# YyzHarry/imbalanced-regression

Measured on NVIDIA H100. Metric: images/sec, higher is better.
Workload: dtype bf16

## Files before the change

### imbalanced-regression_b200/csrc/conv_igemm.cu

```cuda
#include <stdlib.h>
#include "common.cuh"
#include "tc.cuh"
#include "conv.cuh"

namespace dirb200 {
using namespace tc;

constexpr int BM = 128;
constexpr int BK = 64;
constexpr int kProducerThreads = 128;
constexpr int kThreads = 384;
constexpr int kMaxTaps = 25;
constexpr int kMaxSmemBytes = 232448;

struct IgemmParams {
  const __nv_bfloat16* src;
  int n, hs, ws, cs;
  int hm, wm;
  int kh, kw, stride, pad;
  int transposed;
  int cls_on, cls_py, cls_px, full_h, full_w;
  int ntaps_c;
  int tap_list[kMaxTaps];
  long long tap_eoff[kMaxTaps];
  unsigned short tap_r[kMaxTaps], tap_s[kMaxTaps];
  FastDiv fd_hw, fd_wm, fd_cpb, fd_kw, fd_ntiles, fd_persplit;
  int cpb;
  long long pixels;
  int num_kblocks;
  int kblocks_per_split;
  int total_chunks;
  int m_tiles, n_tiles;
  int num_tiles;
  int a_mode;
  int i2c_stride, i2c_lo;
  int ldc;
  void* out;
  float* stat_out;
  const float* epi_scale;
  const float* epi_shift;
  const __nv_bfloat16* epi_res;
  int epi_relu;
  const __nv_bfloat16* bst_y;
  const float* bst_scale;
  const float* bst_shift;
};

template <int BN, bool STAGED_EPI>
struct Cfg {
  static constexpr int kABytes = BM * BK * 2;
  static constexpr int kBBytes = BN * BK * 2;
  static constexpr int kStageBytes = kABytes + kBBytes;
  static constexpr int kStages = BN == 128 ? (STAGED_EPI ? 5 : 6) : 8;
  static constexpr int kBarOffset = kStages * kStageBytes;
  static constexpr int kStageRowBytes = BN * 2 + 16;
  static constexpr int kEpiWarpBytes = 16 * kStageRowBytes;
  static constexpr int kEpiOffset = kBarOffset + 256;
  static constexpr int kStatWarpBytes = 2 * BN * 4;
  static constexpr int kStatOffset = kEpiOffset + (STAGED_EPI ? 8 * kEpiWarpBytes : 0);
  static constexpr int kSmemBytes = kStatOffset + (STAGED_EPI ? 8 * kStatWarpBytes : 0) + 1024;
  static_assert(kSmemBytes <= kMaxSmemBytes, "shared memory budget");
};

__device__ __forceinline__ uint32_t pack_pixel(long long p, const IgemmParams& P) {
  if (p >= P.pixels) return 0u;
  uint32_t n, rem, y, x;
  P.fd_hw.divmod(static_cast<uint32_t>(p), n, rem);
  P.fd_wm.divmod(rem, y, x);
  return 0x80000000u | (n << 18) | (y << 9) | x;
}

struct RowPre {
  int nb, yb, xb;
};
__device__ __forceinline__ RowPre row_pre(const IgemmParams& P, uint32_t pk) {
  RowPre rp;
  const int n = (pk >> 18) & 0x1FFF;
  int y = (pk >> 9) & 0x1FF, x = pk & 0x1FF;
  if (P.cls_on) {
    y = 2 * y + P.cls_py;
    x = 2 * x + P.cls_px;
  }
  rp.nb = n * P.hs;
  if (!P.transposed) {
    rp.yb = y * P.stride - P.pad;
    rp.xb = x * P.stride - P.pad;
  } else {
    rp.yb = y + P.pad;
    rp.xb = x + P.pad;
  }
  if (!(pk >> 31)) rp.yb = -(1 << 28);
  return rp;
}

__device__ __forceinline__ const __nv_bfloat16* tap_source(const IgemmParams& P, const RowPre& rp, int r, int s,
                                                           int coff, bool& ok) {
  int hi, wi;
  ok = true;
  if (!P.transposed) {
    hi = rp.yb + r;
    wi = rp.xb + s;
  } else {
    hi = rp.yb - r;
    wi = rp.xb - s;
    if (P.stride == 2) {
      ok = ((hi | wi) & 1) == 0;
      hi >>= 1;
      wi >>= 1;
    }
  }
  ok = ok && static_cast<unsigned>(hi) < static_cast<unsigned>(P.hs) &&
       static_cast<unsigned>(wi) < static_cast<unsigned>(P.ws);
  return ok ? P.src + (static_cast<size_t>(rp.nb + hi) * P.ws + wi) * P.cs + coff : P.src;
}

template <int BN, bool WGRAD, bool STEM, bool ATMA = false, bool AFFINE = false, bool BSTAT = false>
__global__ void __launch_bounds__(kThreads, 1)
igemm_kernel(const __grid_constant__ CUtensorMap tmap_b, const __grid_constant__ CUtensorMap tmap_a,
             const IgemmParams P) {
  using C = Cfg<BN, !WGRAD>;
  static_assert(BN == 64 || BN == 128, "tile width: one m64n64 / m64n128 wgmma per warpgroup and k step");
  static_assert(!ATMA || !STEM, "TMA-fed A operand: not for the stem");
  static_assert(!AFFINE || (!WGRAD && !STEM), "folded-BN epilogue: non-stem fprop GEMMs only");
  static_assert(!BSTAT || (ATMA && !WGRAD && !AFFINE), "BN-backward moments in the epilogue: TMA-fed dgrad GEMMs only");
  extern __shared__ uint8_t smem_raw[];
  const uint32_t smem_base = (smem_u32(smem_raw) + 1023u) & ~1023u;
  uint8_t* const smem_gen = smem_raw + (smem_base - smem_u32(smem_raw));
  const uint32_t bar_base = smem_base + C::kBarOffset;
  auto a_addr = [&](int s) { return smem_base + s * C::kStageBytes; };
  auto b_addr = [&](int s) { return smem_base + s * C::kStageBytes + C::kABytes; };
  constexpr uint32_t nstages = C::kStages;
  auto full_bar = [&](int s) { return bar_base + 8u * s; };
  auto empty_bar = [&](int s) { return bar_base + 8u * (C::kStages + s); };
  const int warp = static_cast<int>(threadIdx.x >> 5), lane = threadIdx.x & 31;

  int tile_first, tile_end, tile_step, fixed_n = 0;
  if constexpr (WGRAD) {
    tile_first = blockIdx.x; tile_end = P.num_tiles; tile_step = gridDim.x;
  } else {
    uint32_t gi, nn;
    P.fd_ntiles.divmod(blockIdx.x, gi, nn);
    fixed_n = static_cast<int>(nn);
    tile_first = static_cast<int>(gi);
    tile_end = P.m_tiles;
    tile_step = static_cast<int>(P.fd_ntiles.div(gridDim.x - 1u - nn)) + 1;
  }
  auto decode_tile = [&](int t, int& split, int& m_tile, int& n_tile, int& kb_begin, int& nk) {
    if constexpr (WGRAD) {
      uint32_t sp, rem, mt, nt;
      P.fd_persplit.divmod(static_cast<uint32_t>(t), sp, rem);
      P.fd_ntiles.divmod(rem, mt, nt);
      split = static_cast<int>(sp);
      m_tile = static_cast<int>(mt);
      n_tile = static_cast<int>(nt);
      kb_begin = split * P.kblocks_per_split;
      const int kb_end = min(P.num_kblocks, kb_begin + P.kblocks_per_split);
      nk = max(0, kb_end - kb_begin);
    } else {
      split = 0;
      m_tile = t;
      n_tile = fixed_n;
      kb_begin = 0;
      nk = P.num_kblocks;
    }
  };

  if (threadIdx.x == 0) {
    for (int s = 0; s < C::kStages; ++s) {
      mbar_init(full_bar(s), ATMA ? 1 : kProducerThreads + 1);
      mbar_init(empty_bar(s), 8);
    }
    fence_barrier_init();
  }
  __syncthreads();

  if (warp < 4) {
    if constexpr (!ATMA) {
      const int j = lane & 7;
      const int q = lane >> 3;
      uint32_t rs = 0, rph = 0;
      for (int t = tile_first; t < tile_end; t += tile_step) {
        int split, m_tile, n_tile, kb_begin, nk;
        decode_tile(t, split, m_tile, n_tile, kb_begin, nk);
        const int n0 = n_tile * BN;
        long long off8[8];
        uint32_t mask8[8];
        int chunk_r = 0, chunk_s = 0, chunk_c0 = 0;
        bool chunk_ok = true;
        uint32_t tile_off = 0;
        if constexpr (!WGRAD) {
          const RowPre rp = row_pre(P, pack_pixel(static_cast<long long>(m_tile) * BM + warp * 32 + lane, P));
          const bool rvalid = rp.yb > -(1 << 27);
          int oy = rp.yb, ox = rp.xb;
          if (P.transposed && P.stride == 2) { oy >>= 1; ox >>= 1; }
          const long long my_off = (static_cast<long long>(rp.nb + oy) * P.ws + ox) * P.cs;
          uint32_t vy = 0, vx = 0;
          if (rvalid) {
            const int nky = P.kh, nkx = STEM ? 4 : P.kw;
            for (int r = 0; r < nky; ++r) {
              int h = P.transposed ? rp.yb - r : rp.yb + r;
              bool ok = true;
              if (P.transposed && P.stride == 2) { ok = (h & 1) == 0; h >>= 1; }
              vy |= (ok && static_cast<unsigned>(h) < static_cast<unsigned>(P.hs) ? 1u : 0u) << r;
// ... 89 lines not shown
            }
            unsigned long long rowaddr = myaddr;
            if constexpr (STEM)
              rowaddr = reinterpret_cast<unsigned long long>(
                  P.src + ((static_cast<long long>(rp.nb + rp.yb + chunk_r) * P.ws + rp.xb) * P.cs));
#pragma unroll
            for (int i = 0; i < 8; ++i) {
              const int row = 4 * i + q;
              const unsigned long long a = __shfl_sync(0xffffffffu, rowaddr, row);
              const uint32_t okb = __shfl_sync(0xffffffffu, okbits, row);
              const bool ok = STEM ? ((okb >> (j >> 1)) & 1u) : (okb & 1u);
              const __nv_bfloat16* src = reinterpret_cast<const __nv_bfloat16*>(a) + j * 8;
              cp_async16(dst_base + row * 128 + ((j ^ (row & 7)) << 4), ok ? src : P.src, ok ? 16u : 0u);
            }
          }
          if (warp == 0) {
            if (elect_one()) {
              mbar_arrive_expect_tx(full_bar(s), C::kBBytes);
              if constexpr (!WGRAD) {
                tma_load_2d(b_addr(s), &tmap_b, full_bar(s), kcoord * BK, n0);
              } else {
#pragma unroll
                for (int i = 0; i < BN / 64; ++i)
                  tma_load_2d(b_addr(s) + i * 8192, &tmap_b, full_bar(s), n0 + 64 * i, kb * 64);
              }
            }
            __syncwarp();
          }
          cp_async_mbar_arrive_noinc(full_bar(s));
        }
      }
    } else if (warp == 0) {
      uint32_t rs = 0, rph = 0;
      for (int t = tile_first; t < tile_end; t += tile_step) {
        int split, m_tile, n_tile, kb_begin, nk;
        decode_tile(t, split, m_tile, n_tile, kb_begin, nk);
        const int n0 = n_tile * BN;
        int tile_w0 = 0, tile_h0 = 0, tile_n0 = 0;
        if constexpr (!WGRAD) {
          if (P.a_mode == 2) {
            uint32_t tn, rem, y0, x0;
            P.fd_hw.divmod(static_cast<uint32_t>(m_tile) * BM, tn, rem);
            P.fd_wm.divmod(rem, y0, x0);
            tile_n0 = static_cast<int>(tn);
            tile_w0 = static_cast<int>(x0) * P.i2c_stride + P.i2c_lo;
            tile_h0 = static_cast<int>(y0) * P.i2c_stride + P.i2c_lo;
          }
        }
        int tc = 0, cb = 0;
        for (int it = 0; it < nk; ++it) {
          const int s = static_cast<int>(rs);
          mbar_wait(empty_bar(s), rph ^ 1u);
          if (++rs == nstages) { rs = 0; rph ^= 1u; }
          const int kb = kb_begin + it;
          if (elect_one()) {
            if constexpr (!WGRAD) {
              mbar_arrive_expect_tx(full_bar(s), C::kBBytes + C::kABytes);
              if (P.a_mode == 1)
                tma_load_2d(a_addr(s), &tmap_a, full_bar(s), kb * BK, m_tile * BM);
              else
                tma_load_im2col_4d(a_addr(s), &tmap_a, full_bar(s), cb * BK, tile_w0, tile_h0, tile_n0,
                                   P.tap_s[tc], P.tap_r[tc]);
              tma_load_2d(b_addr(s), &tmap_b, full_bar(s), (P.tap_list[tc] * P.cpb + cb) * BK, n0);
            } else {
              const int nchunks = min(2, P.total_chunks - 2 * m_tile);
              mbar_arrive_expect_tx(full_bar(s), C::kBBytes + nchunks * 8192);
// ... 3 lines not shown
              } else {
                uint32_t n0i, rem, y0, x0;
                P.fd_hw.divmod(static_cast<uint32_t>(kb) * 64u, n0i, rem);
                P.fd_wm.divmod(rem, y0, x0);
                for (int i = 0; i < nchunks; ++i) {
                  uint32_t tap, cbk, r, sx;
                  P.fd_cpb.divmod(static_cast<uint32_t>(2 * m_tile + i), tap, cbk);
                  P.fd_kw.divmod(tap, r, sx);
                  tma_load_im2col_4d(a_addr(s) + i * 8192, &tmap_a, full_bar(s), static_cast<int>(cbk) * 64,
                                     static_cast<int>(x0) * P.i2c_stride + P.i2c_lo,
                                     static_cast<int>(y0) * P.i2c_stride + P.i2c_lo, static_cast<int>(n0i),
                                     static_cast<uint16_t>(sx), static_cast<uint16_t>(r));
                }
              }
#pragma unroll
              for (int i = 0; i < BN / 64; ++i)
                tma_load_2d(b_addr(s) + i * 8192, &tmap_b, full_bar(s), n0 + 64 * i, kb * 64);
            }
          }
          if constexpr (!WGRAD) {
            if (++cb == P.cpb) { cb = 0; ++tc; }
          }
          __syncwarp();
        }
      }
    }
    return;
  }

  const int g = (warp >> 2) - 1;
  const int wq = warp & 3;
  const int ew = g * 4 + wq;
  const int fr = lane >> 2, fc = 2 * (lane & 3);
  float* const stat_sm = reinterpret_cast<float*>(smem_gen + C::kStatOffset) + ew * (2 * BN);
  if constexpr (!WGRAD) {
    if (P.stat_out != nullptr)
      for (int i = lane; i < 2 * BN; i += 32) stat_sm[i] = 0.f;
  }
  constexpr uint32_t kLbo = WGRAD ? 8192u : 16u;
  constexpr uint32_t kadv = WGRAD ? (2048u >> 4) : (32u >> 4);
  constexpr int kT = WGRAD ? 1 : 0;
  float acc[BN / 2];
  uint32_t rs = 0, rph = 0;
  for (int t = tile_first; t < tile_end; t += tile_step) {
    int split, m_tile, n_tile, kb_begin, nk;
    decode_tile(t, split, m_tile, n_tile, kb_begin, nk);
    int prev = 0;
    for (int it = 0; it < nk; ++it) {
      const int s = static_cast<int>(rs);
      mbar_wait(full_bar(s), rph);
      if (++rs == nstages) { rs = 0; rph ^= 1u; }
      if constexpr (!ATMA) fence_proxy_async();
      const uint64_t adesc = make_smem_desc(a_addr(s) + g * 8192, kLbo, 1024u);
      const uint64_t bdesc = make_smem_desc(b_addr(s), kLbo, 1024u);
      wgmma_fence_operands(acc);
      wgmma_fence();
#pragma unroll
      for (int k = 0; k < BK / 16; ++k)
        wgmma_bf16<BN, kT, kT>(acc, adesc + static_cast<uint64_t>(k * kadv), bdesc + static_cast<uint64_t>(k * kadv),
                               (it > 0 || k > 0) ? 1u : 0u);
      wgmma_commit();
      wgmma_fence_operands(acc);
      if (it > 0) {
        wgmma_wait<1>();
        if (lane == 0) mbar_arrive(empty_bar(prev));
      }
      prev = s;
    }
    wgmma_wait<0>();
    wgmma_fence_operands(acc);
    if (nk > 0 && lane == 0) mbar_arrive(empty_bar(prev));
    const int n0 = n_tile * BN;

    if constexpr (!WGRAD) {
      const uint32_t stage_base = smem_base + C::kEpiOffset + ew * C::kEpiWarpBytes;
      const bool relu_now = AFFINE && P.epi_relu && P.epi_res == nullptr;
#pragma unroll
      for (int j = 0; j < BN / 8; ++j) {
        const int col = 8 * j + fc;
        float v0 = acc[4 * j], v1 = acc[4 * j + 1], v2 = acc[4 * j + 2], v3 = acc[4 * j + 3];
        if constexpr (AFFINE) {
          const float2 a = __ldg(reinterpret_cast<const float2*>(P.epi_scale + n0 + col));
          const float2 b = __ldg(reinterpret_cast<const float2*>(P.epi_shift + n0 + col));
          v0 = fmaf(v0, a.x, b.x); v1 = fmaf(v1, a.y, b.y); v2 = fmaf(v2, a.x, b.x); v3 = fmaf(v3, a.y, b.y);
          if (relu_now) { v0 = fmaxf(v0, 0.f); v1 = fmaxf(v1, 0.f); v2 = fmaxf(v2, 0.f); v3 = fmaxf(v3, 0.f); }
        }
        __nv_bfloat162 h0 = __floats2bfloat162_rn(v0, v1), h1 = __floats2bfloat162_rn(v2, v3);
        asm volatile("st.shared.b32 [%0], %1;" ::"r"(stage_base + fr * C::kStageRowBytes + col * 2),
                     "r"(*reinterpret_cast<uint32_t*>(&h0)) : "memory");
        asm volatile("st.shared.b32 [%0], %1;" ::"r"(stage_base + (fr + 8) * C::kStageRowBytes + col * 2),
                     "r"(*reinterpret_cast<uint32_t*>(&h1)) : "memory");
      }
      __syncwarp();
      constexpr int kLanesPerRow = BN * 2 / 16;
      constexpr int kRowsPerIter = 32 / kLanesPerRow;
      constexpr int kIters = 16 / kRowsPerIter;
      const int sub = lane / kLanesPerRow, col16 = lane % kLanesPerRow;
      const long long p0 = static_cast<long long>(m_tile) * BM + g * 64 + wq * 16;
      __nv_bfloat16* out_cols = reinterpret_cast<__nv_bfloat16*>(P.out) + n0 + col16 * 8;
#pragma unroll
      for (int i = 0; i < kIters; ++i) {
        const int rl = i * kRowsPerIter + sub;
        const long long p = p0 + rl;
        int orow = (p < P.pixels && nk > 0) ? static_cast<int>(p) : -1;
        if (orow >= 0 && P.cls_on) {
          const uint32_t pk = pack_pixel(p, P);
          const int n = (pk >> 18) & 0x1FFF, yy = (pk >> 9) & 0x1FF, xx = pk & 0x1FF;
          orow = (n * P.full_h + 2 * yy + P.cls_py) * P.full_w + 2 * xx + P.cls_px;
        }
        if (orow >= 0) {
          uint4 val;
          asm volatile("ld.shared.v4.b32 {%0, %1, %2, %3}, [%4];"
                       : "=r"(val.x), "=r"(val.y), "=r"(val.z), "=r"(val.w)
                       : "r"(stage_base + rl * C::kStageRowBytes + col16 * 16));
          if constexpr (AFFINE) {
            if (P.epi_res != nullptr) {
              const uint4 rv = *reinterpret_cast<const uint4*>(P.epi_res + n0 + col16 * 8 + static_cast<long long>(orow) * P.ldc);
              uint32_t o[4] = {val.x, val.y, val.z, val.w};
              const uint32_t rr[4] = {rv.x, rv.y, rv.z, rv.w};
#pragma unroll
              for (int e = 0; e < 4; ++e) {
                float lo = __uint_as_float(o[e] << 16) + __uint_as_float(rr[e] << 16);
                float hi = __uint_as_float(o[e] & 0xffff0000u) + __uint_as_float(rr[e] & 0xffff0000u);
                if (P.epi_relu) { lo = fmaxf(lo, 0.f); hi = fmaxf(hi, 0.f); }
                __nv_bfloat162 h = __floats2bfloat162_rn(lo, hi);
                o[e] = *reinterpret_cast<uint32_t*>(&h);
              }
              val = make_uint4(o[0], o[1], o[2], o[3]);
            }
          }
          *reinterpret_cast<uint4*>(out_cols + static_cast<long long>(orow) * P.ldc) = val;
        }
      }
      if (BSTAT || P.stat_out != nullptr) {
#pragma unroll
        for (int h = 0; h < BN / 64; ++h) {
          const int col = 2 * (lane + 32 * h);
          float s0 = 0.f, s1 = 0.f, q0 = 0.f, q1 = 0.f;
          float2 bsc = make_float2(0.f, 0.f), bsh = bsc;
          if constexpr (BSTAT) {
            bsc = __ldg(reinterpret_cast<const float2*>(P.bst_scale + n0 + col));
            bsh = __ldg(reinterpret_cast<const float2*>(P.bst_shift + n0 + col));
          }
#pragma unroll
          for (int r = 0; r < 16; ++r) {
            uint32_t w;
            asm volatile("ld.shared.b32 %0, [%1];" : "=r"(w) : "r"(stage_base + r * C::kStageRowBytes + col * 2));
            float g0 = __uint_as_float(w << 16), g1 = __uint_as_float(w & 0xffff0000u);
            if constexpr (BSTAT) {
              const long long p = p0 + r;
              const uint32_t yw = p < P.pixels ? __ldg(reinterpret_cast<const unsigned int*>(P.bst_y + p * P.ldc + n0 + col)) : 0u;
              const float y0 = __uint_as_float(yw << 16), y1 = __uint_as_float(yw & 0xffff0000u);
              if (!(fmaf(y0, bsc.x, bsh.x) > 0.f)) g0 = 0.f;
              if (!(fmaf(y1, bsc.y, bsh.y) > 0.f)) g1 = 0.f;
              s0 += g0; s1 += g1;
              q0 = fmaf(g0, y0, q0); q1 = fmaf(g1, y1, q1);
            } else {
              s0 += g0; s1 += g1;
              q0 = fmaf(g0, g0, q0); q1 = fmaf(g1, g1, q1);
            }
          }
          stat_sm[col] += s0;
          stat_sm[col + 1] += s1;
          stat_sm[BN + col] += q0;
          stat_sm[BN + col + 1] += q1;
        }
      }
      __syncwarp();
    } else {
      const int ktot = P.total_chunks * 64;
      const int krow = m_tile * BM + g * 64 + wq * 16 + fr;
      float* out = reinterpret_cast<float*>(P.out) + (static_cast<size_t>(split) * P.ldc + n0) * ktot;
#pragma unroll
      for (int j = 0; j < BN / 8; ++j) {
        const size_t c0 = static_cast<size_t>(8 * j + fc) * ktot;
#pragma unroll
        for (int e = 0; e < 2; ++e) {
          if (krow < ktot) out[c0 + e * ktot + krow] = nk > 0 ? acc[4 * j + e] : 0.f;
          if (krow + 8 < ktot) out[c0 + e * ktot + krow + 8] = nk > 0 ? acc[4 * j + 2 + e] : 0.f;
        }
      }
    }
  }
  if constexpr (!WGRAD) {
    if (P.stat_out != nullptr) {
      asm volatile("bar.sync 1, 256;" ::: "memory");
      const float* all = reinterpret_cast<const float*>(smem_gen + C::kStatOffset);
      float* dst = P.stat_out + static_cast<size_t>(blockIdx.x) * 2 * P.ldc + fixed_n * BN;
      for (int o = static_cast<int>(threadIdx.x) - kProducerThreads; o < 2 * BN; o += kThreads - kProducerThreads) {
        const int k = o / BN, col = o - k * BN;
        const float v = ((all[o] + all[2 * BN + o]) + (all[4 * BN + o] + all[6 * BN + o])) +
                        ((all[8 * BN + o] + all[10 * BN + o]) + (all[12 * BN + o] + all[14 * BN + o]));
        dst[static_cast<size_t>(k) * P.ldc + col] = v;
      }
    }
  }
}

typedef CUresult (*EncodeTiledFn)(CUtensorMap*, CUtensorMapDataType, cuuint32_t, void*, const cuuint64_t*,
                                  const cuuint64_t*, const cuuint32_t*, const cuuint32_t*, CUtensorMapInterleave,
                                  CUtensorMapSwizzle, CUtensorMapL2promotion, CUtensorMapFloatOOBfill);

static EncodeTiledFn encode_fn() {
  static EncodeTiledFn fn = nullptr;
  if (!fn) {
    void* p = nullptr;
    cudaDriverEntryPointQueryResult q;
    if (cudaGetDriverEntryPoint("cuTensorMapEncodeTiled", &p, cudaEnableDefault, &q) == cudaSuccess &&
        q == cudaDriverEntryPointSuccess)
      fn = reinterpret_cast<EncodeTiledFn>(p);
  }
  return fn;
}

int make_tmap_bf16_2d(CUtensorMap* tm, const void* ptr, uint64_t inner, uint64_t outer, uint64_t row_stride_bytes,
                      uint32_t box_outer) {
  EncodeTiledFn fn = encode_fn();
  if (!fn) {
    set_error("cuTensorMapEncodeTiled entry point not available");
// ... 56 lines not shown
  Q.fd_hw = make_fastdiv(static_cast<uint32_t>(Q.hm * Q.wm));
  Q.fd_wm = make_fastdiv(static_cast<uint32_t>(Q.wm));
  Q.fd_cpb = make_fastdiv(static_cast<uint32_t>(Q.cpb > 0 ? Q.cpb : 1));
  Q.fd_kw = make_fastdiv(static_cast<uint32_t>(Q.kw > 0 ? Q.kw : 1));
  Q.fd_ntiles = make_fastdiv(static_cast<uint32_t>(Q.n_tiles > 0 ? Q.n_tiles : 1));
  Q.fd_persplit = make_fastdiv(static_cast<uint32_t>(Q.m_tiles * Q.n_tiles > 0 ? Q.m_tiles * Q.n_tiles : 1));
  const int nt = Q.ntaps_c < kMaxTaps ? Q.ntaps_c : kMaxTaps;
  for (int i = 0; i < kMaxTaps; ++i) {
    Q.tap_eoff[i] = 0;
    Q.tap_r[i] = Q.tap_s[i] = 0;
  }
  for (int i = 0; i < nt && Q.kw > 0; ++i) {
    const int tp = Q.tap_list[i];
    int r = tp / Q.kw, sx = tp - r * Q.kw;
    if (Q.transposed && Q.cls_on) {
      Q.tap_r[i] = static_cast<unsigned short>((Q.cls_py + Q.pad - r) / 2 - Q.i2c_lo);
      Q.tap_s[i] = static_cast<unsigned short>((Q.cls_px + Q.pad - sx) / 2 - Q.i2c_lo);
      r >>= 1; sx >>= 1;
      Q.tap_eoff[i] = -static_cast<long long>(r * Q.ws + sx) * Q.cs;
    } else if (Q.transposed) {
      Q.tap_r[i] = static_cast<unsigned short>(Q.kh - 1 - r);
      Q.tap_s[i] = static_cast<unsigned short>(Q.kw - 1 - sx);
      if (Q.stride == 2) { r >>= 1; sx >>= 1; }
      Q.tap_eoff[i] = -static_cast<long long>(r * Q.ws + sx) * Q.cs;
    } else {
      Q.tap_r[i] = static_cast<unsigned short>(r);
      Q.tap_s[i] = static_cast<unsigned short>(sx);
      Q.tap_eoff[i] = static_cast<long long>(r * Q.ws + sx) * Q.cs;
    }
  }
  return Q;
}

template <int BN, bool WGRAD, bool STEM, bool ATMA = false, bool AFFINE = false, bool BSTAT = false>
static int launch_igemm_impl(const CUtensorMap& tm, const CUtensorMap& tma, const IgemmParams& Qin, cudaStream_t st) {
  using C = Cfg<BN, !WGRAD>;
  const IgemmParams Q = finish_params(Qin);
  static bool configured = false;
  if (!configured) {
    DIRB_CUDA(cudaFuncSetAttribute(igemm_kernel<BN, WGRAD, STEM, ATMA, AFFINE, BSTAT>,
                                   cudaFuncAttributeMaxDynamicSharedMemorySize, C::kSmemBytes));
    configured = true;
  }
  int grid = Q.num_tiles < num_sms() ? Q.num_tiles : num_sms();
  if (!WGRAD && grid < Q.n_tiles) grid = Q.n_tiles;
  t_last_layout = StatLayout{grid, Q.n_tiles, BN, 1};
  igemm_kernel<BN, WGRAD, STEM, ATMA, AFFINE, BSTAT><<<grid, kThreads, C::kSmemBytes, st>>>(tm, tma, Q);
  DIRB_LAUNCHED();
  return DIRB200_OK;
}

template <int BN, bool WGRAD, bool STEM>
static int launch_igemm(const CUtensorMap& tm, const IgemmParams& P, int m_tiles, int splits, cudaStream_t st,
                        const CUtensorMap* tma = nullptr) {
  IgemmParams Q = P;
  Q.m_tiles = m_tiles;
  Q.num_tiles = m_tiles * P.n_tiles * splits;
  if constexpr (!STEM) {
    if (tma) {
      if constexpr (!WGRAD) {
        if (Q.epi_scale != nullptr) return launch_igemm_impl<BN, false, false, true, true>(tm, *tma, Q, st);
        if (Q.bst_y != nullptr) return launch_igemm_impl<BN, false, false, true, false, true>(tm, *tma, Q, st);
      }
      return launch_igemm_impl<BN, WGRAD, false, true>(tm, *tma, Q, st);
    }
  }
  if constexpr (!WGRAD && !STEM) {
    if (Q.epi_scale != nullptr) return launch_igemm_impl<BN, false, false, false, true>(tm, tm, Q, st);
  }
  if (Q.epi_scale != nullptr || Q.bst_y != nullptr) {
    set_error("conv: the BN-backward moments epilogue needs a TMA-fed A operand; the folded-BN one a non-stem fprop");
    return DIRB200_ERR_ARG;
  }
  return launch_igemm_impl<BN, WGRAD, STEM>(tm, tm, Q, st);
}

static int pick_bn(int n_dim) { return n_dim % 128 == 0 ? 128 : 64; }

#define DISPATCH_BN(bn, WG, ST, ...) \
  ((bn) == 128 ? launch_igemm<128, WG, ST>(__VA_ARGS__) : launch_igemm<64, WG, ST>(__VA_ARGS__))

static int check_shape(const ConvShape& s, bool stem, const char* who) {
  DIRB_CHECK_ARG(s.n > 0 && s.h > 0 && s.w > 0 && s.kh > 0 && s.kw > 0 && s.stride > 0 && s.pad >= 0,
                 "%s: bad conv shape", who);
  DIRB_CHECK_ARG(s.cout % 64 == 0, "%s: Cout must be a multiple of 64 (got %d)", who, s.cout);
  DIRB_CHECK_ARG(static_cast<long long>(s.n) * s.h * s.w < (1LL << 31) && static_cast<long long>(s.n) * s.ho * s.wo < (1LL << 31),
                 "%s: more than 2^31 pixels", who);
  if (stem)
    DIRB_CHECK_ARG(s.cin == 16 && s.kh == 4 && s.kw == 4 && s.stride == 1, "%s: stem expects the 4x4x16 s2d form", who);
  else
    DIRB_CHECK_ARG(s.cin % 64 == 0, "%s: Cin must be a multiple of 64 (got %d)", who, s.cin);
  return DIRB200_OK;
}

static bool atma_enabled() {
  static const bool on = [] {
    const char* e = getenv("DIRB200_ATMA");
    return !(e != nullptr && e[0] == '0');
  }();
  return on;
}
static bool is_plain_gemm(const ConvShape& s, bool stem) {
  return !stem && s.kh == 1 && s.kw == 1 && s.stride == 1 && s.pad == 0 && atma_enabled();
}
static bool im2col_enabled() {
  static const bool on = [] {
    const char* e = getenv("DIRB200_IM2COL");
    return !(e != nullptr && e[0] == '0');
  }();
  return on && atma_enabled();
// ... 3 lines not shown
                           cudaStream_t st, float* stat_partial, const ConvEpilogue* epi);

int conv_fprop(const __nv_bfloat16* x, const __nv_bfloat16* w, __nv_bfloat16* y, const ConvShape& s, bool stem,
               cudaStream_t st, float* stat_partial, StatLayout* layout) {
  const int rc = conv_fprop_impl(x, w, y, s, stem, st, stat_partial, nullptr);
  if (layout) *layout = t_last_layout;
  return rc;
}

int conv_fprop_affine(const __nv_bfloat16* x, const __nv_bfloat16* w, __nv_bfloat16* out, const ConvShape& s,
                      const ConvEpilogue& epi, cudaStream_t st) {
  DIRB_CHECK_ARG(epi.scale && epi.shift, "conv_fprop_affine: scale / shift missing");
  return conv_fprop_impl(x, w, out, s, false, st, nullptr, &epi);
}

static int conv_fprop_impl(const __nv_bfloat16* x, const __nv_bfloat16* w, __nv_bfloat16* y, const ConvShape& s, bool stem,
                           cudaStream_t st, float* stat_partial, const ConvEpilogue* epi) {
  if (int rc = check_shape(s, stem, "conv_fprop")) return rc;
  const int ktot = s.kh * s.kw * s.cin;
  IgemmParams P{};
  P.src = x; P.n = s.n; P.hs = s.h; P.ws = s.w; P.cs = s.cin; P.hm = s.ho; P.wm = s.wo;
  P.kh = s.kh; P.kw = s.kw; P.stride = s.stride; P.pad = s.pad; P.transposed = 0;
  P.cpb = stem ? 1 : s.cin / 64;
  P.pixels = static_cast<long long>(s.n) * s.ho * s.wo;
  P.num_kblocks = ktot / 64;
  P.ntaps_c = s.kh * s.kw;
  DIRB_CHECK_ARG(stem || P.ntaps_c <= kMaxTaps, "conv_fprop: at most %d filter taps (got %dx%d)", kMaxTaps, s.kh, s.kw);
  for (int i = 0; i < kMaxTaps; ++i) P.tap_list[i] = i;
  P.ldc = s.cout; P.out = y;
  P.stat_out = stat_partial;
  if (epi) {
    P.epi_scale = epi->scale; P.epi_shift = epi->shift; P.epi_res = epi->residual; P.epi_relu = epi->relu ? 1 : 0;
  }
  const int m_tiles = static_cast<int>((P.pixels + BM - 1) / BM);
  const int bn = pick_bn(s.cout);
  P.n_tiles = s.cout / bn;
  CUtensorMap tm, ta;
  bool tma_fed = false;
  if (is_plain_gemm(s, stem)) {
    if (int rc = make_tmap_bf16_2d(&ta, x, s.cin, static_cast<uint64_t>(P.pixels), static_cast<uint64_t>(s.cin) * 2, BM))
      return rc;
    P.a_mode = 1;
    tma_fed = true;
  } else if (!stem && im2col_enabled()) {
    if (int rc = make_tmap_im2col_bf16(&ta, x, s.cin, s.w, s.h, s.n, -s.pad, -s.pad, s.pad - (s.kw - 1),
                                       s.pad - (s.kh - 1), s.stride, BM))
      return rc;
    P.a_mode = 2; P.i2c_stride = s.stride; P.i2c_lo = -s.pad;
    tma_fed = true;
  }
  if (int rc = make_tmap_bf16_2d(&tm, w, ktot, s.cout, static_cast<uint64_t>(ktot) * 2, bn)) return rc;
  if (stem) return DISPATCH_BN(bn, false, true, tm, P, m_tiles, 1, st);
  if (tma_fed) return DISPATCH_BN(bn, false, false, tm, P, m_tiles, 1, st, &ta);
  return DISPATCH_BN(bn, false, false, tm, P, m_tiles, 1, st);
}

bool conv_dgrad_fuses_bn_moments(const ConvShape& s) {
  return s.stride == 1 && (is_plain_gemm(s, false) || (im2col_enabled() && s.kh == s.kw));
}

int conv_dgrad(const __nv_bfloat16* dy, const __nv_bfloat16* wt, __nv_bfloat16* dx, const ConvShape& s,
               cudaStream_t st, const DgradBnMoments* bnm) {
  if (int rc = check_shape(s, false, "conv_dgrad")) return rc;
  DIRB_CHECK_ARG(!bnm || (conv_dgrad_fuses_bn_moments(s) && bnm->y && bnm->scale && bnm->shift && bnm->partial),
                 "conv_dgrad: BN-backward moments are fused into TMA-fed stride-1 dgrads only");
  DIRB_CHECK_ARG(s.stride == 1 || s.stride == 2, "conv_dgrad: stride must be 1 or 2 (got %d)", s.stride);
  DIRB_CHECK_ARG(s.kh * s.kw <= (s.stride == 1 ? kMaxTaps : 9), "conv_dgrad: at most %d filter taps (stride 2: 9; got %dx%d)",
                 kMaxTaps, s.kh, s.kw);
  const int ktot = s.kh * s.kw * s.cout;
  IgemmParams P{};
  P.src = dy; P.n = s.n; P.hs = s.ho; P.ws = s.wo; P.cs = s.cout; P.hm = s.h; P.wm = s.w;
  P.kh = s.kh; P.kw = s.kw; P.stride = s.stride; P.pad = s.pad; P.transposed = 1;
  P.cpb = s.cout / 64;
  P.ldc = s.cin; P.out = dx;
  if (bnm) {
    P.bst_y = bnm->y; P.bst_scale = bnm->scale; P.bst_shift = bnm->shift; P.stat_out = bnm->partial;
  }
  const int bn = pick_bn(s.cin);
  CUtensorMap tm;
  if (int rc = make_tmap_bf16_2d(&tm, wt, ktot, s.cin, static_cast<uint64_t>(ktot) * 2, bn)) return rc;
  if (s.stride == 1) {
    P.pixels = static_cast<long long>(s.n) * s.h * s.w;
    P.ntaps_c = s.kh * s.kw;
    for (int i = 0; i < kMaxTaps; ++i) P.tap_list[i] = i;
    P.num_kblocks = ktot / 64;
    const int m_tiles = static_cast<int>((P.pixels + BM - 1) / BM);
    P.n_tiles = s.cin / bn;
    CUtensorMap ta;
    bool tma_fed = false;
    if (is_plain_gemm(s, false)) {
      if (int rc = make_tmap_bf16_2d(&ta, dy, s.cout, static_cast<uint64_t>(P.pixels), static_cast<uint64_t>(s.cout) * 2, BM))
        return rc;
      P.a_mode = 1;
      tma_fed = true;
    } else if (im2col_enabled() && s.kh == s.kw) {
      const int lo = s.pad - (s.kh - 1);
      if (int rc = make_tmap_im2col_bf16(&ta, dy, s.cout, s.wo, s.ho, s.n, lo, lo, lo + s.w - s.wo, lo + s.h - s.ho, 1, BM))
        return rc;
      P.a_mode = 2; P.i2c_stride = 1; P.i2c_lo = lo;
      tma_fed = true;
    }
    const int rc = tma_fed ? DISPATCH_BN(bn, false, false, tm, P, m_tiles, 1, st, &ta)
                           : DISPATCH_BN(bn, false, false, tm, P, m_tiles, 1, st);
    if (bnm && bnm->layout) *bnm->layout = t_last_layout;
    return rc;
  }
  bool need_zero = false;
  for (int cls = 0; cls < 4; ++cls) {
    const int py = cls >> 1, px = cls & 1;
    int nt = 0;
    for (int r = 0; r < s.kh; ++r)
      for (int q = 0; q < s.kw; ++q)
        if (((py + s.pad - r) & 1) == 0 && ((px + s.pad - q) & 1) == 0) ++nt;
    if (nt == 0) need_zero = true;
  }
  if (need_zero)
    DIRB_CUDA(cudaMemsetAsync(dx, 0, static_cast<size_t>(s.n) * s.h * s.w * s.cin * sizeof(__nv_bfloat16), st));
  for (int cls = 0; cls < 4; ++cls) {
    IgemmParams Q = P;
    Q.cls_on = 1; Q.cls_py = cls >> 1; Q.cls_px = cls & 1; Q.full_h = s.h; Q.full_w = s.w;
    Q.hm = (s.h - Q.cls_py + 1) / 2;
    Q.wm = (s.w - Q.cls_px + 1) / 2;
    Q.ntaps_c = 0;
    for (int r = 0; r < s.kh; ++r)
      for (int q = 0; q < s.kw; ++q)
        if (((Q.cls_py + s.pad - r) & 1) == 0 && ((Q.cls_px + s.pad - q) & 1) == 0) Q.tap_list[Q.ntaps_c++] = r * s.kw + q;
    if (Q.ntaps_c == 0 || Q.hm <= 0 || Q.wm <= 0) continue;
    Q.pixels = static_cast<long long>(s.n) * Q.hm * Q.wm;
    Q.num_kblocks = Q.ntaps_c * Q.cpb;
    const int m_tiles = static_cast<int>((Q.pixels + BM - 1) / BM);
    Q.n_tiles = s.cin / bn;
    if (im2col_enabled()) {
      int lo = 1 << 20;
      for (int i = 0; i < Q.ntaps_c; ++i) {
        const int r = Q.tap_list[i] / s.kw, q = Q.tap_list[i] % s.kw;
        const int orr = (Q.cls_py + s.pad - r) / 2, oq = (Q.cls_px + s.pad - q) / 2;
        lo = orr < lo ? orr : lo;
        lo = oq < lo ? oq : lo;
      }
      CUtensorMap ta;
      if (int rc = make_tmap_im2col_bf16(&ta, dy, s.cout, s.wo, s.ho, s.n, lo, lo, lo + Q.wm - s.wo, lo + Q.hm - s.ho, 1, BM))
        return rc;
      Q.a_mode = 2; Q.i2c_stride = 1; Q.i2c_lo = lo;
      if (int rc = DISPATCH_BN(bn, false, false, tm, Q, m_tiles, 1, st, &ta)) return rc;
      continue;
    }
    if (int rc = DISPATCH_BN(bn, false, false, tm, Q, m_tiles, 1, st)) return rc;
  }
  return DIRB200_OK;
}

static int wgrad_bn(const ConvShape& s) { return pick_bn(s.cout); }

int conv_wgrad_splits(const ConvShape& s) {
  const long long pixels = static_cast<long long>(s.n) * s.ho * s.wo;
  const int kblocks = static_cast<int>((pixels + 63) / 64);
  const int chunks = s.kh * s.kw * s.cin / 64;
  const int bn = wgrad_bn(s);
  const int m_tiles = (chunks + 1) / 2;
  const int tiles = m_tiles * (s.cout / bn);
  const int sms = num_sms();
  int max_splits = (kblocks + 7) / 8;
  if (max_splits < 1) max_splits = 1;
  int hi = (4 * sms + tiles - 1) / tiles;
  if (hi > max_splits) hi = max_splits;
  int best = 1;
  long long best_cost = -1;
  for (int sp = 1; sp <= hi; ++sp) {
    const long long waves = (static_cast<long long>(tiles) * sp + sms - 1) / sms;
    const long long per = (kblocks + sp - 1) / sp;
    const long long cost = waves * (per + 6);
    if (best_cost < 0 || cost < best_cost) {
      best_cost = cost;
      best = sp;
    }
  }
  return best;
}

size_t conv_wgrad_workspace_bytes(const ConvShape& s) {
// ... 82 lines not shown
```

Baseline: 7673.

## Add 192-row tiles with three consumer warpgroups for TMA-fed fprop/dgrad GEMMs

Adds a three-consumer-warpgroup variant of the implicit-GEMM kernel. A CTA processes 192 output rows per pass, made of 64-row halves drawn from its persistent 128-row tile list, so each loaded B tile is shared by three A blocks instead of two. The variant is chosen automatically for large TMA-fed forward and data-gradient convolutions, and an environment variable can force the tile size. In exchange it uses fewer pipeline stages, a more complex half-tile scheduler with barrier-serialised statistics accumulation, and more threads per CTA.

```diff
diff --git a/imbalanced-regression_b200/csrc/conv_igemm.cu b/imbalanced-regression_b200/csrc/conv_igemm.cu
--- a/imbalanced-regression_b200/csrc/conv_igemm.cu
+++ b/imbalanced-regression_b200/csrc/conv_igemm.cu
@@ -6,10 +6,9 @@
 namespace dirb200 {
 using namespace tc;
 
-constexpr int BM = 128;
 constexpr int BK = 64;
 constexpr int kProducerThreads = 128;
-constexpr int kThreads = 384;
+constexpr int threads_for(int wgs) { return kProducerThreads + 128 * wgs; }
 constexpr int kMaxTaps = 25;
 constexpr int kMaxSmemBytes = 232448;
 
@@ -46,21 +45,25 @@
   const float* bst_shift;
 };
 
-template <int BN, bool STAGED_EPI>
+template <int BN, bool STAGED_EPI, int WGS = 2>
 struct Cfg {
-  static constexpr int kABytes = BM * BK * 2;
+  static constexpr int kBM = 64 * WGS;
+  static constexpr int kEpiWarps = 4 * WGS;
+  static constexpr int kABytes = kBM * BK * 2;
   static constexpr int kBBytes = BN * BK * 2;
   static constexpr int kStageBytes = kABytes + kBBytes;
-  static constexpr int kStages = BN == 128 ? (STAGED_EPI ? 5 : 6) : 8;
+  static constexpr int kStages = WGS == 2 ? (BN == 128 ? (STAGED_EPI ? 5 : 6) : 8) : (BN == 128 ? 4 : 6);
   static constexpr int kBarOffset = kStages * kStageBytes;
   static constexpr int kStageRowBytes = BN * 2 + 16;
   static constexpr int kEpiWarpBytes = 16 * kStageRowBytes;
   static constexpr int kEpiOffset = kBarOffset + 256;
   static constexpr int kStatWarpBytes = 2 * BN * 4;
-  static constexpr int kStatOffset = kEpiOffset + (STAGED_EPI ? 8 * kEpiWarpBytes : 0);
+  static constexpr int kStatOffset = kEpiOffset + (STAGED_EPI ? kEpiWarps * kEpiWarpBytes : 0);
   static constexpr int kSmemBytes = kStatOffset + (STAGED_EPI ? 8 * kStatWarpBytes : 0) + 1024;
   static_assert(kSmemBytes <= kMaxSmemBytes, "shared memory budget");
 };
+static_assert(Cfg<128, true, 3>::kSmemBytes == 225536 && Cfg<64, true, 3>::kSmemBytes == 229632,
+              "192-row tiles: 4 (BN = 128) / 6 (BN = 64) ring stages next to 12 staging tiles and 8 statistics slots");
 
 __device__ __forceinline__ uint32_t pack_pixel(long long p, const IgemmParams& P) {
   if (p >= P.pixels) return 0u;
@@ -114,12 +117,16 @@
   return ok ? P.src + (static_cast<size_t>(rp.nb + hi) * P.ws + wi) * P.cs + coff : P.src;
 }
 
-template <int BN, bool WGRAD, bool STEM, bool ATMA = false, bool AFFINE = false, bool BSTAT = false>
-__global__ void __launch_bounds__(kThreads, 1)
+template <int BN, bool WGRAD, bool STEM, bool ATMA = false, bool AFFINE = false, bool BSTAT = false, int WGS = 2>
+__global__ void __launch_bounds__(threads_for(WGS), 1)
 igemm_kernel(const __grid_constant__ CUtensorMap tmap_b, const __grid_constant__ CUtensorMap tmap_a,
              const IgemmParams P) {
-  using C = Cfg<BN, !WGRAD>;
+  using C = Cfg<BN, !WGRAD, WGS>;
+  constexpr int BM = C::kBM;
+  constexpr int kThreads = threads_for(WGS);
   static_assert(BN == 64 || BN == 128, "tile width: one m64n64 / m64n128 wgmma per warpgroup and k step");
+  static_assert(WGS == 2 || (WGS == 3 && ATMA && !WGRAD),
+                "192-row tiles: TMA-fed fprop / dgrad only (the gather and wgrad producers serve 128 rows)");
   static_assert(!ATMA || !STEM, "TMA-fed A operand: not for the stem");
   static_assert(!AFFINE || (!WGRAD && !STEM), "folded-BN epilogue: non-stem fprop GEMMs only");
   static_assert(!BSTAT || (ATMA && !WGRAD && !AFFINE), "BN-backward moments in the epilogue: TMA-fed dgrad GEMMs only");
@@ -164,11 +171,14 @@
       nk = P.num_kblocks;
     }
   };
+  const int n_halves = WGS == 3 && tile_first < tile_end ? 2 * ((tile_end - tile_first + tile_step - 1) / tile_step) : 0;
+  auto half_row = [&](int i) { return 128LL * (tile_first + (i >> 1) * tile_step) + 64 * (i & 1); };
+  auto half_valid = [&](int i) { return i < n_halves && half_row(i) < P.pixels; };
 
   if (threadIdx.x == 0) {
     for (int s = 0; s < C::kStages; ++s) {
       mbar_init(full_bar(s), ATMA ? 1 : kProducerThreads + 1);
-      mbar_init(empty_bar(s), 8);
+      mbar_init(empty_bar(s), C::kEpiWarps);
     }
     fence_barrier_init();
   }
@@ -324,6 +334,48 @@
       }
     } else if (warp == 0) {
       uint32_t rs = 0, rph = 0;
+      if constexpr (WGS == 3) {
+        const int n0 = fixed_n * BN;
+        for (int i0 = 0; i0 < n_halves; i0 += 3) {
+          int nv = 0, hr[3] = {0, 0, 0}, hw[3] = {0, 0, 0}, hh[3] = {0, 0, 0}, hn[3] = {0, 0, 0};
+#pragma unroll
+          for (int q = 0; q < 3; ++q) {
+            if (!half_valid(i0 + q)) continue;
+            ++nv;
+            hr[q] = static_cast<int>(half_row(i0 + q));
+            if (P.a_mode == 2) {
+              uint32_t tn, rem, y0, x0;
+              P.fd_hw.divmod(static_cast<uint32_t>(hr[q]), tn, rem);
+              P.fd_wm.divmod(rem, y0, x0);
+              hn[q] = static_cast<int>(tn);
+              hw[q] = static_cast<int>(x0) * P.i2c_stride + P.i2c_lo;
+              hh[q] = static_cast<int>(y0) * P.i2c_stride + P.i2c_lo;
+            }
+          }
+          int tc = 0, cb = 0;
+          for (int it = 0; it < P.num_kblocks; ++it) {
+            const int s = static_cast<int>(rs);
+            mbar_wait(empty_bar(s), rph ^ 1u);
+            if (++rs == nstages) { rs = 0; rph ^= 1u; }
+            if (elect_one()) {
+              mbar_arrive_expect_tx(full_bar(s), C::kBBytes + nv * 8192);
+#pragma unroll
+              for (int q = 0; q < 3; ++q) {
+                if (q >= nv) break;
+                if (P.a_mode == 1)
+                  tma_load_2d(a_addr(s) + q * 8192, &tmap_a, full_bar(s), it * BK, hr[q]);
+                else
+                  tma_load_im2col_4d(a_addr(s) + q * 8192, &tmap_a, full_bar(s), cb * BK, hw[q], hh[q], hn[q],
+                                     P.tap_s[tc], P.tap_r[tc]);
+              }
+              tma_load_2d(b_addr(s), &tmap_b, full_bar(s), (P.tap_list[tc] * P.cpb + cb) * BK, n0);
+            }
+            if (++cb == P.cpb) { cb = 0; ++tc; }
+            __syncwarp();
+          }
+        }
+        return;
+      }
       for (int t = tile_first; t < tile_end; t += tile_step) {
         int split, m_tile, n_tile, kb_begin, nk;
         decode_tile(t, split, m_tile, n_tile, kb_begin, nk);
@@ -393,21 +445,34 @@
   const int wq = warp & 3;
   const int ew = g * 4 + wq;
   const int fr = lane >> 2, fc = 2 * (lane & 3);
-  float* const stat_sm = reinterpret_cast<float*>(smem_gen + C::kStatOffset) + ew * (2 * BN);
+  float* const stat_base = reinterpret_cast<float*>(smem_gen + C::kStatOffset);
   if constexpr (!WGRAD) {
-    if (P.stat_out != nullptr)
-      for (int i = lane; i < 2 * BN; i += 32) stat_sm[i] = 0.f;
+    if (P.stat_out != nullptr && ew < 8)
+      for (int i = lane; i < 2 * BN; i += 32) stat_base[ew * 2 * BN + i] = 0.f;
   }
   constexpr uint32_t kLbo = WGRAD ? 8192u : 16u;
   constexpr uint32_t kadv = WGRAD ? (2048u >> 4) : (32u >> 4);
   constexpr int kT = WGRAD ? 1 : 0;
   float acc[BN / 2];
   uint32_t rs = 0, rph = 0;
-  for (int t = tile_first; t < tile_end; t += tile_step) {
+  const int item_first = WGS == 3 ? 0 : tile_first, item_step = WGS == 3 ? 1 : tile_step;
+  const int item_end = WGS == 3 ? (n_halves + 2) / 3 : tile_end;
+  for (int t = item_first; t < item_end; t += item_step) {
     int split, m_tile, n_tile, kb_begin, nk;
     decode_tile(t, split, m_tile, n_tile, kb_begin, nk);
+    const bool valid = WGS == 2 || half_valid(3 * t + g);
+    const long long row0 = WGS == 2 ? static_cast<long long>(m_tile) * BM + g * 64 : half_row(3 * t + g);
+    float* const stat_sm = stat_base + ((WGS == 2 ? g : (3 * t + g) & 1) * 4 + wq) * (2 * BN);
+    if (!valid) {
+      for (int it = 0; it < nk; ++it) {
+        const int s = static_cast<int>(rs);
+        mbar_wait(full_bar(s), rph);
+        if (++rs == nstages) { rs = 0; rph ^= 1u; }
+        if (lane == 0) mbar_arrive(empty_bar(s));
+      }
+    }
     int prev = 0;
-    for (int it = 0; it < nk; ++it) {
+    for (int it = 0; it < (valid ? nk : 0); ++it) {
       const int s = static_cast<int>(rs);
       mbar_wait(full_bar(s), rph);
       if (++rs == nstages) { rs = 0; rph ^= 1u; }
@@ -430,70 +495,72 @@
     }
     wgmma_wait<0>();
     wgmma_fence_operands(acc);
-    if (nk > 0 && lane == 0) mbar_arrive(empty_bar(prev));
+    if (valid && nk > 0 && lane == 0) mbar_arrive(empty_bar(prev));
     const int n0 = n_tile * BN;
 
     if constexpr (!WGRAD) {
       const uint32_t stage_base = smem_base + C::kEpiOffset + ew * C::kEpiWarpBytes;
-      const bool relu_now = AFFINE && P.epi_relu && P.epi_res == nullptr;
-#pragma unroll
-      for (int j = 0; j < BN / 8; ++j) {
-        const int col = 8 * j + fc;
-        float v0 = acc[4 * j], v1 = acc[4 * j + 1], v2 = acc[4 * j + 2], v3 = acc[4 * j + 3];
-        if constexpr (AFFINE) {
-          const float2 a = __ldg(reinterpret_cast<const float2*>(P.epi_scale + n0 + col));
-          const float2 b = __ldg(reinterpret_cast<const float2*>(P.epi_shift + n0 + col));
-          v0 = fmaf(v0, a.x, b.x); v1 = fmaf(v1, a.y, b.y); v2 = fmaf(v2, a.x, b.x); v3 = fmaf(v3, a.y, b.y);
-          if (relu_now) { v0 = fmaxf(v0, 0.f); v1 = fmaxf(v1, 0.f); v2 = fmaxf(v2, 0.f); v3 = fmaxf(v3, 0.f); }
+      const long long p0 = row0 + wq * 16;
+      if (valid) {
+        const bool relu_now = AFFINE && P.epi_relu && P.epi_res == nullptr;
+#pragma unroll
+        for (int j = 0; j < BN / 8; ++j) {
+          const int col = 8 * j + fc;
+          float v0 = acc[4 * j], v1 = acc[4 * j + 1], v2 = acc[4 * j + 2], v3 = acc[4 * j + 3];
+          if constexpr (AFFINE) {
+            const float2 a = __ldg(reinterpret_cast<const float2*>(P.epi_scale + n0 + col));
+            const float2 b = __ldg(reinterpret_cast<const float2*>(P.epi_shift + n0 + col));
+            v0 = fmaf(v0, a.x, b.x); v1 = fmaf(v1, a.y, b.y); v2 = fmaf(v2, a.x, b.x); v3 = fmaf(v3, a.y, b.y);
+            if (relu_now) { v0 = fmaxf(v0, 0.f); v1 = fmaxf(v1, 0.f); v2 = fmaxf(v2, 0.f); v3 = fmaxf(v3, 0.f); }
+          }
+          __nv_bfloat162 h0 = __floats2bfloat162_rn(v0, v1), h1 = __floats2bfloat162_rn(v2, v3);
+          asm volatile("st.shared.b32 [%0], %1;" ::"r"(stage_base + fr * C::kStageRowBytes + col * 2),
+                       "r"(*reinterpret_cast<uint32_t*>(&h0)) : "memory");
+          asm volatile("st.shared.b32 [%0], %1;" ::"r"(stage_base + (fr + 8) * C::kStageRowBytes + col * 2),
+                       "r"(*reinterpret_cast<uint32_t*>(&h1)) : "memory");
         }
-        __nv_bfloat162 h0 = __floats2bfloat162_rn(v0, v1), h1 = __floats2bfloat162_rn(v2, v3);
-        asm volatile("st.shared.b32 [%0], %1;" ::"r"(stage_base + fr * C::kStageRowBytes + col * 2),
-                     "r"(*reinterpret_cast<uint32_t*>(&h0)) : "memory");
-        asm volatile("st.shared.b32 [%0], %1;" ::"r"(stage_base + (fr + 8) * C::kStageRowBytes + col * 2),
-                     "r"(*reinterpret_cast<uint32_t*>(&h1)) : "memory");
-      }
-      __syncwarp();
-      constexpr int kLanesPerRow = BN * 2 / 16;
-      constexpr int kRowsPerIter = 32 / kLanesPerRow;
-      constexpr int kIters = 16 / kRowsPerIter;
-      const int sub = lane / kLanesPerRow, col16 = lane % kLanesPerRow;
-      const long long p0 = static_cast<long long>(m_tile) * BM + g * 64 + wq * 16;
-      __nv_bfloat16* out_cols = reinterpret_cast<__nv_bfloat16*>(P.out) + n0 + col16 * 8;
-#pragma unroll
-      for (int i = 0; i < kIters; ++i) {
-        const int rl = i * kRowsPerIter + sub;
-        const long long p = p0 + rl;
-        int orow = (p < P.pixels && nk > 0) ? static_cast<int>(p) : -1;
-        if (orow >= 0 && P.cls_on) {
-          const uint32_t pk = pack_pixel(p, P);
-          const int n = (pk >> 18) & 0x1FFF, yy = (pk >> 9) & 0x1FF, xx = pk & 0x1FF;
-          orow = (n * P.full_h + 2 * yy + P.cls_py) * P.full_w + 2 * xx + P.cls_px;
-        }
-        if (orow >= 0) {
-          uint4 val;
-          asm volatile("ld.shared.v4.b32 {%0, %1, %2, %3}, [%4];"
-                       : "=r"(val.x), "=r"(val.y), "=r"(val.z), "=r"(val.w)
-                       : "r"(stage_base + rl * C::kStageRowBytes + col16 * 16));
-          if constexpr (AFFINE) {
-            if (P.epi_res != nullptr) {
-              const uint4 rv = *reinterpret_cast<const uint4*>(P.epi_res + n0 + col16 * 8 + static_cast<long long>(orow) * P.ldc);
-              uint32_t o[4] = {val.x, val.y, val.z, val.w};
-              const uint32_t rr[4] = {rv.x, rv.y, rv.z, rv.w};
-#pragma unroll
-              for (int e = 0; e < 4; ++e) {
-                float lo = __uint_as_float(o[e] << 16) + __uint_as_float(rr[e] << 16);
-                float hi = __uint_as_float(o[e] & 0xffff0000u) + __uint_as_float(rr[e] & 0xffff0000u);
-                if (P.epi_relu) { lo = fmaxf(lo, 0.f); hi = fmaxf(hi, 0.f); }
-                __nv_bfloat162 h = __floats2bfloat162_rn(lo, hi);
-                o[e] = *reinterpret_cast<uint32_t*>(&h);
+        __syncwarp();
+        constexpr int kLanesPerRow = BN * 2 / 16;
+        constexpr int kRowsPerIter = 32 / kLanesPerRow;
+        constexpr int kIters = 16 / kRowsPerIter;
+        const int sub = lane / kLanesPerRow, col16 = lane % kLanesPerRow;
+        __nv_bfloat16* out_cols = reinterpret_cast<__nv_bfloat16*>(P.out) + n0 + col16 * 8;
+#pragma unroll
+        for (int i = 0; i < kIters; ++i) {
+          const int rl = i * kRowsPerIter + sub;
+          const long long p = p0 + rl;
+          int orow = (p < P.pixels && nk > 0) ? static_cast<int>(p) : -1;
+          if (orow >= 0 && P.cls_on) {
+            const uint32_t pk = pack_pixel(p, P);
+            const int n = (pk >> 18) & 0x1FFF, yy = (pk >> 9) & 0x1FF, xx = pk & 0x1FF;
+            orow = (n * P.full_h + 2 * yy + P.cls_py) * P.full_w + 2 * xx + P.cls_px;
+          }
+          if (orow >= 0) {
+            uint4 val;
+            asm volatile("ld.shared.v4.b32 {%0, %1, %2, %3}, [%4];"
+                         : "=r"(val.x), "=r"(val.y), "=r"(val.z), "=r"(val.w)
+                         : "r"(stage_base + rl * C::kStageRowBytes + col16 * 16));
+            if constexpr (AFFINE) {
+              if (P.epi_res != nullptr) {
+                const uint4 rv = *reinterpret_cast<const uint4*>(P.epi_res + n0 + col16 * 8 + static_cast<long long>(orow) * P.ldc);
+                uint32_t o[4] = {val.x, val.y, val.z, val.w};
+                const uint32_t rr[4] = {rv.x, rv.y, rv.z, rv.w};
+#pragma unroll
+                for (int e = 0; e < 4; ++e) {
+                  float lo = __uint_as_float(o[e] << 16) + __uint_as_float(rr[e] << 16);
+                  float hi = __uint_as_float(o[e] & 0xffff0000u) + __uint_as_float(rr[e] & 0xffff0000u);
+                  if (P.epi_relu) { lo = fmaxf(lo, 0.f); hi = fmaxf(hi, 0.f); }
+                  __nv_bfloat162 h = __floats2bfloat162_rn(lo, hi);
+                  o[e] = *reinterpret_cast<uint32_t*>(&h);
+                }
+                val = make_uint4(o[0], o[1], o[2], o[3]);
               }
-              val = make_uint4(o[0], o[1], o[2], o[3]);
-            }
-          }
-          *reinterpret_cast<uint4*>(out_cols + static_cast<long long>(orow) * P.ldc) = val;
+            }
+            *reinterpret_cast<uint4*>(out_cols + static_cast<long long>(orow) * P.ldc) = val;
+          }
         }
       }
-      if (BSTAT || P.stat_out != nullptr) {
+      auto add_stats = [&]() {
 #pragma unroll
         for (int h = 0; h < BN / 64; ++h) {
           const int col = 2 * (lane + 32 * h);
@@ -526,6 +593,14 @@
           stat_sm[BN + col] += q0;
           stat_sm[BN + col + 1] += q1;
         }
+      };
+      if constexpr (WGS == 2) {
+        if (BSTAT || P.stat_out != nullptr) add_stats();
+      } else if (P.stat_out != nullptr) {
+        asm volatile("bar.sync 1, %0;" ::"n"(kThreads - kProducerThreads) : "memory");
+        if (valid && g != 2) add_stats();
+        asm volatile("bar.sync 1, %0;" ::"n"(kThreads - kProducerThreads) : "memory");
+        if (valid && g == 2) add_stats();
       }
       __syncwarp();
     } else {
@@ -545,7 +620,7 @@
   }
   if constexpr (!WGRAD) {
     if (P.stat_out != nullptr) {
-      asm volatile("bar.sync 1, 256;" ::: "memory");
+      asm volatile("bar.sync 1, %0;" ::"n"(kThreads - kProducerThreads) : "memory");
       const float* all = reinterpret_cast<const float*>(smem_gen + C::kStatOffset);
       float* dst = P.stat_out + static_cast<size_t>(blockIdx.x) * 2 * P.ldc + fixed_n * BN;
       for (int o = static_cast<int>(threadIdx.x) - kProducerThreads; o < 2 * BN; o += kThreads - kProducerThreads) {
@@ -668,39 +743,54 @@
   return Q;
 }
 
-template <int BN, bool WGRAD, bool STEM, bool ATMA = false, bool AFFINE = false, bool BSTAT = false>
+template <int BN, bool WGRAD, bool STEM, bool ATMA = false, bool AFFINE = false, bool BSTAT = false, int WGS = 2>
 static int launch_igemm_impl(const CUtensorMap& tm, const CUtensorMap& tma, const IgemmParams& Qin, cudaStream_t st) {
-  using C = Cfg<BN, !WGRAD>;
+  using C = Cfg<BN, !WGRAD, WGS>;
   const IgemmParams Q = finish_params(Qin);
   static bool configured = false;
   if (!configured) {
-    DIRB_CUDA(cudaFuncSetAttribute(igemm_kernel<BN, WGRAD, STEM, ATMA, AFFINE, BSTAT>,
+    DIRB_CUDA(cudaFuncSetAttribute(igemm_kernel<BN, WGRAD, STEM, ATMA, AFFINE, BSTAT, WGS>,
                                    cudaFuncAttributeMaxDynamicSharedMemorySize, C::kSmemBytes));
     configured = true;
   }
   int grid = Q.num_tiles < num_sms() ? Q.num_tiles : num_sms();
   if (!WGRAD && grid < Q.n_tiles) grid = Q.n_tiles;
   t_last_layout = StatLayout{grid, Q.n_tiles, BN, 1};
-  igemm_kernel<BN, WGRAD, STEM, ATMA, AFFINE, BSTAT><<<grid, kThreads, C::kSmemBytes, st>>>(tm, tma, Q);
+  igemm_kernel<BN, WGRAD, STEM, ATMA, AFFINE, BSTAT, WGS><<<grid, threads_for(WGS), C::kSmemBytes, st>>>(tm, tma, Q);
   DIRB_LAUNCHED();
   return DIRB200_OK;
 }
 
 template <int BN, bool WGRAD, bool STEM>
 static int launch_igemm(const CUtensorMap& tm, const IgemmParams& P, int m_tiles, int splits, cudaStream_t st,
-                        const CUtensorMap* tma = nullptr) {
+                        const CUtensorMap* tma = nullptr, int bm = 128) {
   IgemmParams Q = P;
   Q.m_tiles = m_tiles;
   Q.num_tiles = m_tiles * P.n_tiles * splits;
   if constexpr (!STEM) {
     if (tma) {
       if constexpr (!WGRAD) {
+        if (bm == 192) {
+          if constexpr (BN == 64) {
+            if (Q.bst_y != nullptr) return launch_igemm_impl<BN, false, false, true, false, true, 3>(tm, *tma, Q, st);
+          }
+          if (Q.bst_y != nullptr) {
+            set_error("conv: BN-backward moments at BN = 128 need 128-row tiles");
+            return DIRB200_ERR_ARG;
+          }
+          if (Q.epi_scale != nullptr) return launch_igemm_impl<BN, false, false, true, true, false, 3>(tm, *tma, Q, st);
+          return launch_igemm_impl<BN, false, false, true, false, false, 3>(tm, *tma, Q, st);
+        }
         if (Q.epi_scale != nullptr) return launch_igemm_impl<BN, false, false, true, true>(tm, *tma, Q, st);
         if (Q.bst_y != nullptr) return launch_igemm_impl<BN, false, false, true, false, true>(tm, *tma, Q, st);
       }
       return launch_igemm_impl<BN, WGRAD, false, true>(tm, *tma, Q, st);
     }
   }
+  if (bm != 128) {
+    set_error("conv: 192-row tiles need a TMA-fed fprop / dgrad");
+    return DIRB200_ERR_ARG;
+  }
   if constexpr (!WGRAD && !STEM) {
     if (Q.epi_scale != nullptr) return launch_igemm_impl<BN, false, false, false, true>(tm, tm, Q, st);
   }
@@ -712,6 +802,17 @@
 }
 
 static int pick_bn(int n_dim) { return n_dim % 128 == 0 ? 128 : 64; }
+
+static int tile_rows_forced() {
+  const char* e = getenv("DIRB200_TILE_ROWS");
+  const int r = e != nullptr ? atoi(e) : 0;
+  return r == 128 || r == 192 ? r : 0;
+}
+
+static int pick_bm(long long pixels, int n_tiles) {
+  if (int f = tile_rows_forced()) return f;
+  return (pixels + 127) / 128 * n_tiles >= 2LL * num_sms() ? 192 : 128;
+}
 
 #define DISPATCH_BN(bn, WG, ST, ...) \
   ((bn) == 128 ? launch_igemm<128, WG, ST>(__VA_ARGS__) : launch_igemm<64, WG, ST>(__VA_ARGS__))
@@ -781,26 +882,25 @@
   if (epi) {
     P.epi_scale = epi->scale; P.epi_shift = epi->shift; P.epi_res = epi->residual; P.epi_relu = epi->relu ? 1 : 0;
   }
-  const int m_tiles = static_cast<int>((P.pixels + BM - 1) / BM);
   const int bn = pick_bn(s.cout);
   P.n_tiles = s.cout / bn;
+  const bool plain = is_plain_gemm(s, stem), tma_fed = plain || (!stem && im2col_enabled());
+  const int bm = tma_fed ? pick_bm(P.pixels, P.n_tiles) : 128;
+  const int m_tiles = static_cast<int>((P.pixels + 127) / 128), box = bm == 192 ? 64 : 128;
   CUtensorMap tm, ta;
-  bool tma_fed = false;
-  if (is_plain_gemm(s, stem)) {
-    if (int rc = make_tmap_bf16_2d(&ta, x, s.cin, static_cast<uint64_t>(P.pixels), static_cast<uint64_t>(s.cin) * 2, BM))
+  if (plain) {
+    if (int rc = make_tmap_bf16_2d(&ta, x, s.cin, static_cast<uint64_t>(P.pixels), static_cast<uint64_t>(s.cin) * 2, box))
       return rc;
     P.a_mode = 1;
-    tma_fed = true;
-  } else if (!stem && im2col_enabled()) {
+  } else if (tma_fed) {
     if (int rc = make_tmap_im2col_bf16(&ta, x, s.cin, s.w, s.h, s.n, -s.pad, -s.pad, s.pad - (s.kw - 1),
-                                       s.pad - (s.kh - 1), s.stride, BM))
+                                       s.pad - (s.kh - 1), s.stride, box))
       return rc;
     P.a_mode = 2; P.i2c_stride = s.stride; P.i2c_lo = -s.pad;
-    tma_fed = true;
   }
   if (int rc = make_tmap_bf16_2d(&tm, w, ktot, s.cout, static_cast<uint64_t>(ktot) * 2, bn)) return rc;
   if (stem) return DISPATCH_BN(bn, false, true, tm, P, m_tiles, 1, st);
-  if (tma_fed) return DISPATCH_BN(bn, false, false, tm, P, m_tiles, 1, st, &ta);
+  if (tma_fed) return DISPATCH_BN(bn, false, false, tm, P, m_tiles, 1, st, &ta, bm);
   return DISPATCH_BN(bn, false, false, tm, P, m_tiles, 1, st);
 }
 
@@ -833,23 +933,22 @@
     P.ntaps_c = s.kh * s.kw;
     for (int i = 0; i < kMaxTaps; ++i) P.tap_list[i] = i;
     P.num_kblocks = ktot / 64;
-    const int m_tiles = static_cast<int>((P.pixels + BM - 1) / BM);
     P.n_tiles = s.cin / bn;
+    const bool plain = is_plain_gemm(s, false), tma_fed = plain || (im2col_enabled() && s.kh == s.kw);
+    const int bm = tma_fed && !(bnm && bn == 128) ? pick_bm(P.pixels, P.n_tiles) : 128;
+    const int m_tiles = static_cast<int>((P.pixels + 127) / 128), box = bm == 192 ? 64 : 128;
     CUtensorMap ta;
-    bool tma_fed = false;
-    if (is_plain_gemm(s, false)) {
-      if (int rc = make_tmap_bf16_2d(&ta, dy, s.cout, static_cast<uint64_t>(P.pixels), static_cast<uint64_t>(s.cout) * 2, BM))
+    if (plain) {
+      if (int rc = make_tmap_bf16_2d(&ta, dy, s.cout, static_cast<uint64_t>(P.pixels), static_cast<uint64_t>(s.cout) * 2, box))
         return rc;
       P.a_mode = 1;
-      tma_fed = true;
-    } else if (im2col_enabled() && s.kh == s.kw) {
+    } else if (tma_fed) {
       const int lo = s.pad - (s.kh - 1);
-      if (int rc = make_tmap_im2col_bf16(&ta, dy, s.cout, s.wo, s.ho, s.n, lo, lo, lo + s.w - s.wo, lo + s.h - s.ho, 1, BM))
+      if (int rc = make_tmap_im2col_bf16(&ta, dy, s.cout, s.wo, s.ho, s.n, lo, lo, lo + s.w - s.wo, lo + s.h - s.ho, 1, box))
         return rc;
       P.a_mode = 2; P.i2c_stride = 1; P.i2c_lo = lo;
-      tma_fed = true;
-    }
-    const int rc = tma_fed ? DISPATCH_BN(bn, false, false, tm, P, m_tiles, 1, st, &ta)
+    }
+    const int rc = tma_fed ? DISPATCH_BN(bn, false, false, tm, P, m_tiles, 1, st, &ta, bm)
                            : DISPATCH_BN(bn, false, false, tm, P, m_tiles, 1, st);
     if (bnm && bnm->layout) *bnm->layout = t_last_layout;
     return rc;
@@ -877,9 +976,10 @@
     if (Q.ntaps_c == 0 || Q.hm <= 0 || Q.wm <= 0) continue;
     Q.pixels = static_cast<long long>(s.n) * Q.hm * Q.wm;
     Q.num_kblocks = Q.ntaps_c * Q.cpb;
-    const int m_tiles = static_cast<int>((Q.pixels + BM - 1) / BM);
     Q.n_tiles = s.cin / bn;
     if (im2col_enabled()) {
+      const int bm = pick_bm(Q.pixels, Q.n_tiles);
+      const int m_tiles = static_cast<int>((Q.pixels + 127) / 128), box = bm == 192 ? 64 : 128;
       int lo = 1 << 20;
       for (int i = 0; i < Q.ntaps_c; ++i) {
         const int r = Q.tap_list[i] / s.kw, q = Q.tap_list[i] % s.kw;
@@ -888,13 +988,13 @@
         lo = oq < lo ? oq : lo;
       }
       CUtensorMap ta;
-      if (int rc = make_tmap_im2col_bf16(&ta, dy, s.cout, s.wo, s.ho, s.n, lo, lo, lo + Q.wm - s.wo, lo + Q.hm - s.ho, 1, BM))
+      if (int rc = make_tmap_im2col_bf16(&ta, dy, s.cout, s.wo, s.ho, s.n, lo, lo, lo + Q.wm - s.wo, lo + Q.hm - s.ho, 1, box))
         return rc;
       Q.a_mode = 2; Q.i2c_stride = 1; Q.i2c_lo = lo;
-      if (int rc = DISPATCH_BN(bn, false, false, tm, Q, m_tiles, 1, st, &ta)) return rc;
+      if (int rc = DISPATCH_BN(bn, false, false, tm, Q, m_tiles, 1, st, &ta, bm)) return rc;
       continue;
     }
-    if (int rc = DISPATCH_BN(bn, false, false, tm, Q, m_tiles, 1, st)) return rc;
+    if (int rc = DISPATCH_BN(bn, false, false, tm, Q, static_cast<int>((Q.pixels + 127) / 128), 1, st)) return rc;
   }
   return DIRB200_OK;
 }
```

New measurement: 7676 (median of 6 runs). About the same (+0.0%).
